# TheIllusionistMirage/libKPEG

Hardware: NVIDIA B200
Metric: decode_mpixel_per_s (higher is better)
Workload: dtype u8/int16 entropy decode, f32 IDCT (f64 on the exact path)

## Files before the change

### libkpeg_b200/csrc/k3_fused.cu

```cuda
#include <cuda_runtime.h>
#include <stddef.h>
#include <stdint.h>

#include <algorithm>
#include <utility>

#include "entropy_core.h"
#include "idct_core.h"
#include "kernels.cuh"
#include "kpeg_common.h"

namespace kpeg {

template <int NAT>
struct NatZz {
    static constexpr int value = make_zigzag_tables().nat2zz[NAT];
};

#ifndef KPEG_EXACT_SKIP_ZERO
#define KPEG_EXACT_SKIP_ZERO 1
#endif

#ifndef KPEG_EXACT_WIDEN_INT
#define KPEG_EXACT_WIDEN_INT 0
// ... 7 lines not shown
constexpr float COLOUR_SAFE_A = 4.0f * (COLOUR_FAST_RANGE - 8.0f);
constexpr float SAMPLE_SAFE_A = 4.0f * 32000.0f;

constexpr float SAMPLE_MAGIC = RINT_MAGIC + 32768.0f;

__host__ __device__ constexpr int tie_bit(int row, int col) { return ((col & 4) ? 0 : 16) + 15 - (4 * (row & 3) + (col & 3)); }
__device__ __forceinline__ int tie_sample(int w, int b)
{
    const int k = 15 - (b & 15);
    return (4 * w + (k >> 2)) * 8 + ((b & 16) ? 0 : 4) + (k & 3);
}

#ifndef KPEG_IDCT_PREFETCH_AHEAD
#define KPEG_IDCT_PREFETCH_AHEAD 1184
#endif
constexpr uint32_t IDCT_PREFETCH_AHEAD = KPEG_IDCT_PREFETCH_AHEAD;

constexpr int TIE_LIST_CAP = IDCT_TIE_LIST_CAP;
constexpr uint32_t TIE_EMPTY = 0xFFFFFFFFu;

template <int NC>
struct IdctSmem {
    static constexpr int NM = IDCT_MCUS_PER_CTA;
    static constexpr int NB = NM * NC;
    union {
        uint4 coef[NB * 8];
        float4 samp[NC * 8 * 2 * NM];
    };
    float2 qpair[NC][32];
    uint2 tiemask[NB];
    uint16_t ties[TIE_LIST_CAP];
    uint8_t flag[NB];
    uint32_t ntie, any_huge;
    uint32_t img0, by0, bx0, mi0;
    unsigned long long mbar;
};
static_assert(sizeof(IdctSmem<3>) <= (233472 / 8 - 1024), "idct_kernel<3> no longer fits eight CTAs per SM");

struct F2 {
    unsigned long long v;
};
__device__ __forceinline__ F2 pack2(float lo, float hi)
{
    F2 r;
    asm("mov.b64 %0, {%1, %2};" : "=l"(r.v) : "f"(lo), "f"(hi));
    return r;
}
__device__ __forceinline__ void unpack2(F2 a, float &lo, float &hi) { asm("mov.b64 {%0, %1}, %2;" : "=f"(lo), "=f"(hi) : "l"(a.v)); }
__device__ __forceinline__ float lo2(F2 a)
{
    float lo, hi;
    unpack2(a, lo, hi);
    return lo;
}
__device__ __forceinline__ float hi2(F2 a)
{
    float lo, hi;
    unpack2(a, lo, hi);
    return hi;
}
__device__ __forceinline__ F2 splat2(float k) { return pack2(k, k); }
__device__ __forceinline__ F2 lane_add(F2 a, F2 b)
{
    F2 r;
    asm("add.rn.f32x2 %0, %1, %2;" : "=l"(r.v) : "l"(a.v), "l"(b.v));
    return r;
// ... 277 lines not shown
    asm volatile("st.shared.u16 [%0], %1;" ::"r"(addr), "h"((uint16_t)v) : "memory");
}

template <int NC>
__global__ void __launch_bounds__(NC * IDCT_MCUS_PER_CTA, NC == 3 ? KPEG_IDCT_MIN_CTAS : 16) idct_kernel(IdctArgs a)
{
    constexpr int NM = IDCT_MCUS_PER_CTA;
    constexpr int NB = NM * NC;
    extern __shared__ __align__(128) unsigned char smem_raw[];
    IdctSmem<NC> &sm = *reinterpret_cast<IdctSmem<NC> *>(smem_raw);

    const int t = threadIdx.x;
    const int comp = t / NM;
    const int ml = t % NM;
    const int bl = ml * NC + comp;
    const uint32_t total_mcus = a.g.nimages * a.g.mcus_per_image;
    const uint32_t strip = blockIdx.x;
    const uint32_t mcu0 = strip * NM;
    const uint32_t m = mcu0 + ml;
    const bool active = m < total_mcus;

    const uint32_t bar = smem_u32(&sm.mbar);
    if (t == 0) {
        constexpr uint32_t table_bytes = NC * 64u * 4u, tile_bytes = NB * 128u;
        const char *tile = reinterpret_cast<const char *>(a.tiles) + (size_t)strip * tile_bytes;
        mbar_init(bar, 1);
        mbar_expect_tx(bar, table_bytes + tile_bytes);
        bulk_load(smem_u32(sm.coef), tile, tile_bytes, bar);
        bulk_load(smem_u32(sm.qpair), a.tables->qpair, table_bytes, bar);
        if (strip + IDCT_PREFETCH_AHEAD < a.nstrips)
            asm volatile("cp.async.bulk.prefetch.L2.global [%0], %1;" ::"l"(tile + (size_t)IDCT_PREFETCH_AHEAD * tile_bytes), "r"(tile_bytes) : "memory");
        sm.ntie = 0;
        sm.any_huge = 0;
        const uint32_t img = mcu0 / a.g.mcus_per_image, mi = mcu0 - img * a.g.mcus_per_image;
        sm.img0 = img;
        sm.mi0 = mi;
        sm.by0 = mi / a.g.mcus_x;
        sm.bx0 = mi - sm.by0 * a.g.mcus_x;
        mbar_wait(bar, 0);
    }
    __syncthreads();

    uint4 ch[8];
#pragma unroll
    for (int k = 0; k < 8; ++k)
        ch[k] = sm.coef[bl * 8 + (k ^ (bl & 7))];
    __syncthreads();
    uint32_t tie_lo = 0, tie_hi = 0;
    if (active) {
        F2 P[32];
        float a_ac, a_dc;
        dequant_dezigzag(ch, sm.qpair[comp], P, a_ac, a_dc, std::make_integer_sequence<int, 32>{});
        const float A = a_ac + a_dc;
        uint32_t flag = (A != 0.0f ? BLK_NONZERO : 0u) | (A > COLOUR_SAFE_A ? BLK_WIDE : 0u);
        if (A > SAMPLE_SAFE_A) {
            flag |= BLK_HUGE;
            sm.any_huge = 1u;
        } else if (a_ac == 0.0f) {
            const int dcv = (int)(ch[0].x & 0xFFFFu) - (int)COEF_BIAS;
            const int F = dcv * __ldg(&a.tables->qint[comp][0]);
            const float tt = mul_f32(__ldg(&a.tables->cc[0][0]), (float)F);
            const float b = (float)round_half_away(0.25f * tt);
            const float4 row = make_float4(b, b, b, b);
#pragma unroll
            for (int i = 0; i < 16; ++i)
                sm.samp[(comp * 16 + i) * NM + ml] = row;
// ... 124 lines not shown
            uint8_t *dst = img_base + ((size_t)y * W + bx * 8u) * NC;
            if (vec_ok) {
#pragma unroll
                for (int k = 0; k < NC; ++k)
                    reinterpret_cast<uint2 *>(dst)[k] = make_uint2(out[2 * k], out[2 * k + 1]);
            } else {
                const uint32_t nbytes = (full_w ? 8u : W - bx * 8u) * NC;
#pragma unroll
                for (int j = 0; j < 8 * NC; ++j)
                    if ((uint32_t)j < nbytes)
                        dst[j] = (uint8_t)(out[j >> 2] >> (8 * (j & 3)));
            }
            while (redo) {
                const int j = __ffs((int)redo) - 1;
                redo &= redo - 1u;
                if (bx * 8u + (uint32_t)j >= W)
                    continue;
                const float *sp = reinterpret_cast<const float *>(sm.samp);
                const int sy = (int)sp[(((0 * 8 + row) * 2 + (j >> 2)) * NM + ml) * 4 + (j & 3)];
                const int sb = (int)sp[(((1 * 8 + row) * 2 + (j >> 2)) * NM + ml) * 4 + (j & 3)];
                const int sr = (int)sp[((((NC - 1) * 8 + row) * 2 + (j >> 2)) * NM + ml) * 4 + (j & 3)];
                const uint32_t e = colour_exact_int(sy, sb, sr);
                dst[3 * j] = (uint8_t)e;
                dst[3 * j + 1] = (uint8_t)(e >> 8);
                dst[3 * j + 2] = (uint8_t)(e >> 16);
                ++colour_exact;
            }
        }
    }
    __syncthreads();

    const uint32_t ntie = sm.ntie;
    if (ntie == 0u && sm.any_huge == 0u) {
        if (t == 0)
            a.tie_cnt[strip] = 0u;
        if (colour_exact)
            atomicAdd(&a.meta->colour_exact, colour_exact);
        return;
    }
    float *spf = reinterpret_cast<float *>(sm.samp);
    const uint4 *gtiles = reinterpret_cast<const uint4 *>(a.tiles);
    const uint32_t blk0 = mcu0 * (uint32_t)NC;
    auto samp_index = [&](uint32_t c, uint32_t mm_l, int s) {
        return ((((c * 8u + (uint32_t)(s >> 3)) * 2u + (uint32_t)((s & 7) >> 2)) * NM + mm_l) * 4u) + (uint32_t)(s & 3);
    };
    auto resolve = [&](uint32_t b, int s) {
        const uint32_t c = b % NC, mm_l = b / NC;
        const int e = exact_sample_global<NC>(gtiles, a.tables, blk0 + b, c, s);
        spf[samp_index(c, mm_l, s)] = (float)e;
    };
    auto repaint = [&](uint32_t b, int s) {
        const uint32_t mm_l = b / NC;
        if (mcu0 + mm_l >= total_mcus)
            return;
        uint32_t img, by, bx;
        mcu_origin(mm_l, img, by, bx);
        const uint32_t px = bx * 8u + (uint32_t)(s & 7), py = by * 8u + (uint32_t)(s >> 3);
        if (px >= W || py >= H)
            return;
        const int y = (int)spf[samp_index(0, mm_l, s)];
        int cb = 0, cr = 0;
        if (NC == 3) {
            cb = (int)spf[samp_index(1, mm_l, s)];
            cr = (int)spf[samp_index(NC - 1, mm_l, s)];
        }
        const uint32_t v = colour_px<NC>(y, cb, cr);
        uint8_t *dst = a.pixels + ((size_t)img * W * H + (size_t)py * W + px) * NC;
        dst[0] = (uint8_t)v;
        if (NC == 3) {
            dst[1] = (uint8_t)(v >> 8);
            dst[2] = (uint8_t)(v >> 16);
        }
    };
    if (ntie <= (uint32_t)TIE_LIST_CAP) {
        for (uint32_t i = (uint32_t)t; i < ntie; i += (uint32_t)NB) {
            const uint32_t e = sm.ties[i], b = e & 127u, mm_l = b / NC, c = b % NC;
            const int sidx = (int)(e >> 7);
            const int tbit = tie_bit(sidx >> 3, sidx & 7);
            uint32_t flags = 0, huge = 0;
#pragma unroll
            for (int cc = 0; cc < NC; ++cc) {
                const uint2 tm = sm.tiemask[mm_l * NC + cc];
                flags |= ((((sidx >> 3) & 4) ? tm.y : tm.x) >> tbit & 1u) << cc;
                huge |= sm.flag[mm_l * NC + cc];
            }
            uint4 r = make_uint4(TIE_EMPTY, 0, 0, 0);
            uint32_t img, by, bx;
            mcu_origin(mm_l, img, by, bx);
            const uint32_t px = bx * 8u + (uint32_t)(sidx & 7), py = by * 8u + (uint32_t)(sidx >> 3);
            if ((flags & (0u - flags)) == (1u << c) && !(huge & BLK_HUGE) && mcu0 + mm_l < total_mcus && px < W && py < H) {
                r.x = img * W * H + py * W + px;
                r.y = mcu0 + mm_l;
                auto biased = [&](uint32_t c) { return ((uint32_t)(int)spf[samp_index(c, mm_l, sidx)] + COEF_BIAS) & 0xFFFFu; };
                r.z = (uint32_t)sidx | (flags << 8) | (biased(0) << 16);
                r.w = NC == 3 ? biased(1) | (biased(2) << 16) : 0u;
            }
            a.tie_rec[(size_t)strip * TIE_LIST_CAP + i] = r;
        }
        if (t == 0)
            a.tie_cnt[strip] = ntie;
    } else {
        if (t == 0)
            a.tie_cnt[strip] = 0u;
        for (int pass = 0; pass < 2; ++pass) {
            uint32_t lo = tie_lo, hi = tie_hi;
            while (lo | hi) {
                int w, b;
                if (lo) {
                    w = 0;
                    b = __ffs((int)lo) - 1;
                    lo &= lo - 1u;
                } else {
                    w = 1;
                    b = __ffs((int)hi) - 1;
                    hi &= hi - 1u;
                }
                if (pass == 0)
                    resolve((uint32_t)bl, tie_sample(w, b));
                else
                    repaint((uint32_t)bl, tie_sample(w, b));
            }
            __syncthreads();
        }
    }
    if (sm.any_huge) {
        __syncthreads();
        for (uint32_t i = (uint32_t)t; i < (uint32_t)NM * 64u; i += (uint32_t)NB) {
            const uint32_t mm_l = i >> 6;
            const int s = (int)(i & 63u);
            uint32_t fl = 0;
            for (int c = 0; c < NC; ++c)
                fl |= sm.flag[mm_l * NC + c];
            if (!(fl & BLK_HUGE) || mcu0 + mm_l >= total_mcus)
                continue;
            uint32_t img, by, bx;
            mcu_origin(mm_l, img, by, bx);
// ... 8 lines not shown
            dst[0] = (uint8_t)v;
            if (NC == 3) {
                dst[1] = (uint8_t)(v >> 8);
                dst[2] = (uint8_t)(v >> 16);
            }
        }
    }
    if (t == 0)
        atomicAdd(&a.meta->exact_samples, ntie);
    if (colour_exact)
        atomicAdd(&a.meta->colour_exact, colour_exact);
}

template <int NC>
__device__ __noinline__ int exact_sample_global(const uint4 *tiles, const DeviceTables *T, uint32_t gb, uint32_t comp, int s)
{
    uint4 ch[8];
#pragma unroll
    for (int k = 0; k < 8; ++k)
        ch[k] = __ldg(tiles + coef_tile_chunk(gb, (uint32_t)k));
    const int x = s >> 3, y = s & 7;
    double cx[8], cy[8];
#pragma unroll
    for (int k = 0; k < 8; ++k) {
        cx[k] = __ldg(&T->cosd[x][k]);
        cy[k] = __ldg(&T->cosd[y][k]);
    }
    const float sum = exact_terms(ch, T->qint[comp], cx, cy, __ldg(&T->cc[0][0]), __ldg(&T->cc[0][1]),
                                  std::make_integer_sequence<int, 64>{});
    const float out = (float)mul_f64(0.25, (double)sum);
    return round_half_away(out);
}

constexpr int PATCH_WARPS = 8;

template <int NC>
__global__ void __launch_bounds__(PATCH_WARPS * 32) idct_patch_kernel(IdctArgs a)
{
    const uint32_t lane = threadIdx.x & 31u, wl = threadIdx.x >> 5;
    const uint4 *tiles = reinterpret_cast<const uint4 *>(a.tiles);
    for (uint32_t s0 = blockIdx.x * 32u; s0 < a.nstrips; s0 += gridDim.x * 32u) {
        const uint32_t strip = s0 + lane;
        const uint32_t cnt = strip < a.nstrips ? min(__ldg(a.tie_cnt + strip), (uint32_t)TIE_LIST_CAP) : 0u;
        uint32_t incl = cnt;
#pragma unroll
        for (int d = 1; d < 32; d <<= 1) {
            const uint32_t o = __shfl_up_sync(0xffffffffu, incl, d);
            if ((int)lane >= d)
                incl += o;
        }
        const uint32_t total = __shfl_sync(0xffffffffu, incl, 31);
        for (uint32_t e0 = wl * 32u; e0 < total; e0 += PATCH_WARPS * 32u) {
            const uint32_t e = e0 + lane;
            uint32_t lo = 0;
#pragma unroll
            for (int step = 16; step >= 1; step >>= 1) {
                const uint32_t v = __shfl_sync(0xffffffffu, incl, (int)(lo + (uint32_t)step - 1u));
                if (v <= e)
                    lo += (uint32_t)step;
            }
            const uint32_t before = __shfl_sync(0xffffffffu, incl - cnt, (int)min(lo, 31u));
            if (e >= total)
                continue;
            const uint4 r = __ldg(a.tie_rec + (size_t)(s0 + lo) * TIE_LIST_CAP + (e - before));
            if (r.x == TIE_EMPTY)
                continue;
            const int s = (int)(r.z & 63u);
            const uint32_t flags = (r.z >> 8) & 7u;
            int v[3] = {(int)(r.z >> 16) - (int)COEF_BIAS, (int)(r.w & 0xFFFFu) - (int)COEF_BIAS, (int)(r.w >> 16) - (int)COEF_BIAS};
            for (uint32_t left = flags; left != 0u; left &= left - 1u) {
                const uint32_t c = (uint32_t)__ffs((int)left) - 1u;
                const int ex = exact_sample_global<NC>(tiles, a.tables, r.y * NC + c, c, s);
                v[0] = c == 0u ? ex : v[0];
                v[1] = c == 1u ? ex : v[1];
                v[2] = c == 2u ? ex : v[2];
            }
            const uint32_t px = colour_px<NC>(v[0], v[1], v[2]);
            uint8_t *dst = a.pixels + (size_t)r.x * NC;
            dst[0] = (uint8_t)px;
            if (NC == 3) {
                dst[1] = (uint8_t)(px >> 8);
                dst[2] = (uint8_t)(px >> 16);
            }
        }
    }
}

void k3_configure()
{
    cudaFuncSetAttribute(idct_kernel<3>, cudaFuncAttributeMaxDynamicSharedMemorySize, (int)sizeof(IdctSmem<3>));
    cudaFuncSetAttribute(idct_kernel<1>, cudaFuncAttributeMaxDynamicSharedMemorySize, (int)sizeof(IdctSmem<1>));
}

uint32_t k3_strip_slots(uint32_t ncomp) { return (uint32_t)IDCT_MCUS_PER_CTA * ncomp * 64u; }

cudaError_t launch_idct(const IdctArgs &a_in, cudaStream_t s, uint32_t *launches)
{
    IdctArgs a = a_in;
    const uint32_t total_mcus = a.g.nimages * a.g.mcus_per_image;
    const uint32_t grid = (total_mcus + IDCT_MCUS_PER_CTA - 1) / IDCT_MCUS_PER_CTA;
    if (a.g.ncomp == 3)
        idct_kernel<3><<<grid, 3 * IDCT_MCUS_PER_CTA, sizeof(IdctSmem<3>), s>>>(a);
    else
        idct_kernel<1><<<grid, IDCT_MCUS_PER_CTA, sizeof(IdctSmem<1>), s>>>(a);
    ++*launches;
    const uint32_t pgrid = std::min<uint32_t>((grid + 31u) / 32u, 148u * 16u);
    if (a.g.ncomp == 3)
        idct_patch_kernel<3><<<pgrid, PATCH_WARPS * 32, 0, s>>>(a);
    else
        idct_patch_kernel<1><<<pgrid, PATCH_WARPS * 32, 0, s>>>(a);
    ++*launches;
    return cudaSuccess;
}

}
```

### libkpeg_b200/csrc/kernels.cuh

```cuda
#ifndef KPEG_KERNELS_CUH
#define KPEG_KERNELS_CUH

#include <cuda_runtime.h>

#include "kpeg_common.h"

namespace kpeg {

constexpr int MAX_RELAY_ROUNDS = 64;

inline int relay_slot(int r) { return r < MAX_RELAY_ROUNDS ? r : 2 + ((r - 2) % (MAX_RELAY_ROUNDS - 2)); }

struct DevMeta {
    uint32_t total_kept;
    uint32_t total_rst;
    uint32_t total_bits;
    uint32_t nsub;
    uint32_t status;
    uint32_t exact_samples;
    uint32_t colour_exact;
    uint32_t final_slot;
    uint32_t reserved_[2];
    uint32_t relay_rounds;
    uint32_t grid_bar;
    uint32_t rec_alt_count;
    uint32_t changed[MAX_RELAY_ROUNDS];
};

struct UnstuffArgs {
    const uint8_t *scan;
    uint32_t scan_len;
    uint32_t ntiles;
    uint32_t *tile_kept, *tile_rst;
    uint32_t *cls;
    uint8_t *words;
    uint32_t *seg_bit;
    uint32_t nseg;
    DevMeta *meta;
};

constexpr int UNSTUFF_THREADS = 256;
constexpr int UNSTUFF_BYTES_PER_THREAD = 16;
constexpr int UNSTUFF_TILE = UNSTUFF_THREADS * UNSTUFF_BYTES_PER_THREAD;

struct EntropyArgs {
    const uint32_t *words;
    const uint32_t *seg_bit;
    const DeviceTables *tables;
    DevMeta *meta;
    SubState *state;
    uint32_t *worklist[2];
    uint32_t *seg_hint;
    uint32_t *start_slot;
    uint2 *scan_tiles;
    long long *scan_tiles_dcs;
// ... 9 lines not shown
    uint32_t *strip_sub;
    uint32_t strip_slots;
    uint32_t nstrips;
    uint32_t nsub_max;
    JobGeom g;
};

constexpr int ENTROPY_THREADS = 128;

constexpr int IDCT_MCUS_PER_CTA = 32;
KPEG_HD uint32_t coef_tile_chunk(uint32_t block, uint32_t k) { return block * 8u + (k ^ (block & 7u)); }
KPEG_HD uint32_t coef_tile_byte(uint32_t slot) { return (slot * 2u) ^ ((slot >> 2) & 0x70u); }

struct ExpandArgs {
    const uint32_t *rec;
    const uint32_t *nrec;
    const uint32_t *rec_alt;
    uint32_t rec_kmax;
    const uint32_t *start_slot;
    const uint32_t *strip_sub;
    const long long *dcpre;
    void *tiles;
    uint32_t nstrips;
    DevMeta *meta;
    JobGeom g;
};

struct IdctArgs {
    const void *tiles;
    uint32_t nstrips;
    const DeviceTables *tables;
    uint8_t *pixels;
    uint4 *tie_rec;
    uint32_t *tie_cnt;
    DevMeta *meta;
    JobGeom g;
};
constexpr int IDCT_TIE_LIST_CAP = 96;


void kernels_context_created();
void kernels_context_destroyed();
void kernels_configure(int max_concurrent_jobs);
void launch_repack_scans(const uint8_t *stage, uint8_t *scan, const uint64_t *ends, uint32_t n, cudaStream_t s);
void launch_write_separators(uint8_t *scan, const uint64_t *ends, uint32_t n, cudaStream_t s);
void launch_count_restart_markers(const uint8_t *scan, uint32_t len, uint32_t *count, cudaStream_t s);
void launch_gray_to_rgb(const uint8_t *gray, uint8_t *rgb, size_t npixels, cudaStream_t s);
void launch_rgb_to_planar(const uint8_t *rgb, uint8_t *planes, size_t npixels, cudaStream_t s);
void launch_unstuff(const UnstuffArgs &a, uint32_t sub_bits, cudaStream_t s, uint32_t *launches);
void launch_entropy_cold(const EntropyArgs &a, cudaStream_t s, uint32_t *launches);
void launch_entropy_relay(const EntropyArgs &a, int round, cudaStream_t s, uint32_t *launches);
cudaError_t launch_entropy_relay_loop(const EntropyArgs &a, int first, int last, cudaStream_t s, uint32_t *launches);
void launch_entropy_scan(const EntropyArgs &a, cudaStream_t s, uint32_t *launches);
void launch_entropy_write(const EntropyArgs &a, cudaStream_t s, uint32_t *launches);
void launch_dc_integrate(const JobGeom &g, const int16_t *dcdiff, int16_t *dc, cudaStream_t s, uint32_t *launches);
void launch_expand(const ExpandArgs &a, cudaStream_t s, uint32_t *launches);
void launch_tiles_from_matrix(const JobGeom &g, const int16_t *coef, const int16_t *dc, void *tiles, cudaStream_t s, uint32_t *launches);
void launch_matrix_from_tiles(const void *tiles, int16_t *coef, uint32_t total_blocks, cudaStream_t s);
void launch_interleave_tiles(const void *t0, const void *t1, const void *t2, void *out, uint32_t nmcu_padded, cudaStream_t s,
                             uint32_t *launches);
cudaError_t launch_idct(const IdctArgs &a, cudaStream_t s, uint32_t *launches);
void k3_configure();
uint32_t k3_strip_slots(uint32_t ncomp);

}
#endif
```

### libkpeg_b200/csrc/kpeg_cuda.cu

```cuda
#include <cuda_runtime.h>
#include <math.h>
#include <stdio.h>
#include <stdlib.h>
#include <string.h>

#include <algorithm>
#include <string>
#include <vector>

#include "host_tables.h"
#include "kernels.cuh"
#include "kpeg_common.h"
#include "kpeg_cuda.h"

using namespace kpeg;

namespace {

struct DevBuf {
    void *p = nullptr;
    size_t cap = 0;
    void *raw = nullptr;
};

// ... 4 lines not shown
    void *p = nullptr;
    size_t cap = 0;
};

constexpr int MAX_EVENTS = 192;
constexpr int NLANES = 8;

struct Copy {
    void *dst;
    const void *src;
    size_t bytes;
    int peer = -1;
};

struct Job {
    bool active = false;
    JobGeom g = {};
    EntropyArgs ea = {};
    ExpandArgs xa = {};
    IdctArgs ia = {};
    int rounds = 0;
    uint32_t launches = 0;
    uint32_t extra_iterations = 0;
    bool use_records = true;
    bool loop_used = true;
    size_t scan_len = 0;
    std::vector<Copy> d2h;
    bool entropy_only = false;
};

struct Lane {
    cudaStream_t stream = nullptr;
    DevBuf scan, words, seg_bit, tile_kept, tile_rst, cls, state, work, seg_hint, start_slot, scan_tiles;
    DevBuf coef, dcdiff, dc, tiles, tie_rec, tie_cnt, pixels, meta, rec, nrec, rec_alt, strip_sub, dcs, dcpre, scan_tiles_dcs;
    PinBuf h_meta;
    PinBuf h_stage, h_ends;
    DevBuf d_ends, d_stage;
    cudaEvent_t ev[MAX_EVENTS] = {};
    int ev_stage[MAX_EVENTS] = {};
    int nev = 0;
    Job job;
};

}

struct kpeg_ctx {
    int device = 0;
    std::string err;
    bool profiling = false;
    uint32_t sub_bits = 512;
    bool sub_bits_auto = true;
    int relay_rounds = 8;
    bool use_records = true;
    int split_parts = 4;
    int host_chunks = 8;
    int submit_parts = 1;
    int band_parts = 4;
    DevBuf band_counts;
    PinBuf h_band_counts;
    bool relay_round2_wide = false;
    bool d2h_chain = true;
    bool d2h_chain_armed = false;
    cudaEvent_t d2h_done = nullptr;
    Lane lane[NLANES];

    DevBuf tables, merged;
    DevBuf scan_tiles[3];
// ... 273 lines not shown
        const uint64_t bits = (uint64_t)scan_len * 8u;
        sub_bits = (bits >= segs * ((uint64_t)4 << 20) && bits >= blocks * 96u) ? 1024u : 512u;
    }
    int rc = make_job_geom(pl, nimages, sub_bits, &g, &why);
    if (rc != KPEG_OK)
        return fail(ctx, rc, why);
    if (scan_len == 0 || scan_len >= (1ull << 29))
        return fail(ctx, KPEG_ERR_ARG, "entropy-coded segment must be 1 byte .. 512 MiB");
    TRY(upload_plan(ctx, pl));

    const uint32_t S = (uint32_t)scan_len;
    const uint32_t ntiles = (S + 15u + UNSTUFF_TILE - 1) / UNSTUFF_TILE;
    const uint32_t nsub_max = (uint32_t)(((uint64_t)S * 8u + g.sub_bits - 1u) / g.sub_bits) + 1u;
    const uint32_t total_mcus = g.nimages * g.mcus_per_image;
    const uint32_t nstrips = (total_mcus + IDCT_MCUS_PER_CTA - 1) / IDCT_MCUS_PER_CTA;
    const size_t words_bytes = ((size_t)S + 3u) / 4u * 4u + 64u;

    TRY(ensure(ctx, s, L.words, words_bytes));
    TRY(ensure(ctx, s, L.seg_bit, ((size_t)g.nseg + 2u) * 4u));
    TRY(ensure(ctx, s, L.tile_kept, (size_t)ntiles * 4u));
    TRY(ensure(ctx, s, L.tile_rst, (size_t)ntiles * 4u));
    TRY(ensure(ctx, s, L.cls, (size_t)ntiles * UNSTUFF_THREADS * 4u));
    TRY(ensure(ctx, s, L.state, (size_t)nsub_max * sizeof(SubState)));
    TRY(ensure(ctx, s, L.work, (size_t)nsub_max * 2u * sizeof(uint32_t)));
    TRY(ensure(ctx, s, L.seg_hint, (size_t)nsub_max * 4u));
    TRY(ensure(ctx, s, L.start_slot, (size_t)nsub_max * 4u));
    TRY(ensure(ctx, s, L.scan_tiles, ((size_t)nsub_max / 1024u + 2u) * sizeof(uint2)));
    TRY(ensure(ctx, s, L.strip_sub, ((size_t)nstrips + 1u) * sizeof(uint32_t)));
    TRY(ensure(ctx, s, L.dcs, (size_t)nsub_max * sizeof(long long)));
    TRY(ensure(ctx, s, L.dcpre, (size_t)nsub_max * sizeof(long long)));
    TRY(ensure(ctx, s, L.scan_tiles_dcs, ((size_t)nsub_max / 1024u + 2u) * sizeof(long long)));
    TRY(ensure(ctx, s, L.tiles, (size_t)nstrips * IDCT_MCUS_PER_CTA * g.ncomp * 128u + 256u));
    TRY(ensure(ctx, s, L.tie_rec, (size_t)nstrips * IDCT_TIE_LIST_CAP * sizeof(uint4)));
    TRY(ensure(ctx, s, L.tie_cnt, (size_t)nstrips * sizeof(uint32_t)));
    TRY(ensure(ctx, s, L.meta, sizeof(DevMeta)));
    TRY(ensure_pinned(ctx, s, L.h_meta, sizeof(DevMeta)));
    const uint32_t rec_kmax = (g.sub_bits * 3u / 8u + 7u) & ~7u;
    const uint32_t rec_alt_cap = nsub_max / 4u + 1024u;
    if (ctx->use_records) {
        TRY(ensure(ctx, s, L.rec, (size_t)rec_kmax * ((size_t)nsub_max / 32u + 1u) * 32u * sizeof(uint32_t)));
        TRY(ensure(ctx, s, L.nrec, (size_t)nsub_max * sizeof(uint32_t)));
        TRY(ensure(ctx, s, L.rec_alt, (size_t)rec_alt_cap * rec_kmax * sizeof(uint32_t)));
    }

    J = Job();
    J.use_records = ctx->use_records && ctx->plan_fits_records;
    J.active = true;
    J.g = g;
    J.scan_len = scan_len;
    J.d2h = std::move(d2h);
    J.entropy_only = tiles_only != nullptr;
    void *const tiles = tiles_only ? tiles_only : L.tiles.p;
    DevMeta *d_meta = (DevMeta *)L.meta.p;

    CK(cudaMemsetAsync(d_meta, 0, sizeof(DevMeta), s));
    mark(ctx, L, KPEG_T_MEMSET);

    UnstuffArgs ua;
    ua.scan = d_scan;
    ua.scan_len = S;
    ua.ntiles = ntiles;
    ua.tile_kept = (uint32_t *)L.tile_kept.p;
    ua.tile_rst = (uint32_t *)L.tile_rst.p;
    ua.cls = (uint32_t *)L.cls.p;
    ua.words = (uint8_t *)L.words.p;
    ua.seg_bit = (uint32_t *)L.seg_bit.p;
    ua.nseg = g.nseg;
// ... 17 lines not shown
    ea.dcpre = (long long *)L.dcpre.p;
    ea.rec = J.use_records ? (uint32_t *)L.rec.p : nullptr;
    ea.nrec = (uint32_t *)L.nrec.p;
    ea.rec_kmax = rec_kmax;
    ea.rec_alt = (uint32_t *)L.rec_alt.p;
    ea.rec_alt_cap = rec_alt_cap;
    ea.coef = nullptr;
    ea.dcdiff = nullptr;
    ea.strip_sub = (uint32_t *)L.strip_sub.p;
    ea.strip_slots = k3_strip_slots(g.ncomp);
    ea.nstrips = nstrips;
    ea.nsub_max = nsub_max;
    ea.g = g;

    ExpandArgs &xa = J.xa;
    xa.rec = ea.rec;
    xa.nrec = ea.nrec;
    xa.rec_alt = ea.rec_alt;
    xa.rec_kmax = rec_kmax;
    xa.start_slot = ea.start_slot;
    xa.strip_sub = ea.strip_sub;
    xa.dcpre = ea.dcpre;
    xa.tiles = tiles;
    xa.nstrips = nstrips;
    xa.meta = d_meta;
    xa.g = g;

    IdctArgs &ia = J.ia;
    ia.tiles = tiles;
    ia.nstrips = nstrips;
    ia.tables = (const DeviceTables *)ctx->tables.p;
    ia.pixels = d_pixels;
    ia.tie_rec = (uint4 *)L.tie_rec.p;
    ia.tie_cnt = (uint32_t *)L.tie_cnt.p;
    ia.meta = d_meta;
    ia.g = g;

    launch_entropy_cold(ea, s, &J.launches);
    mark(ctx, L, KPEG_T_ENTROPY_COLD);
    J.rounds = ctx->relay_rounds < 2 ? 2 : (ctx->relay_rounds > MAX_RELAY_ROUNDS - 1 ? MAX_RELAY_ROUNDS - 1 : ctx->relay_rounds);
    launch_entropy_relay(ea, 1, s, &J.launches);
    mark(ctx, L, KPEG_T_ENTROPY_RELAY);
    if (ctx->relay_round2_wide)
        launch_entropy_relay(ea, 2, s, &J.launches);
    const int loop_first = ctx->relay_round2_wide ? 3 : 2;
    J.rounds = MAX_RELAY_ROUNDS - 2;
    if (launch_entropy_relay_loop(ea, loop_first, J.rounds, s, &J.launches) != cudaSuccess) {
        J.loop_used = false;
        J.rounds = std::max(loop_first, std::min(ctx->relay_rounds, MAX_RELAY_ROUNDS - 1));
        for (int r = loop_first; r <= J.rounds; ++r)
            launch_entropy_relay(ea, r, s, &J.launches);
    }
    mark(ctx, L, KPEG_T_RELAY_SPARSE);
    return enqueue_downstream(ctx, L);
}

struct NamedBuf {
    const char *name;
    DevBuf *buf;
};

int check_guards(kpeg_ctx *ctx, Lane &L)
{
    NamedBuf bufs[] = {{"cls", &L.cls},           {"scan", &L.scan},         {"words", &L.words},       {"seg_bit", &L.seg_bit},
                       {"tile_kept", &L.tile_kept}, {"tile_rst", &L.tile_rst}, {"state", &L.state},       {"work", &L.work},
                       {"seg_hint", &L.seg_hint}, {"start_slot", &L.start_slot}, {"scan_tiles", &L.scan_tiles},
                       {"coef", &L.coef},         {"dcdiff", &L.dcdiff},     {"tiles", &L.tiles},       {"tie_rec", &L.tie_rec},   {"tie_cnt", &L.tie_cnt},     {"strip_sub", &L.strip_sub}, {"dc", &L.dc}, {"dcs", &L.dcs}, {"dcpre", &L.dcpre}, {"scan_tiles_dcs", &L.scan_tiles_dcs}, {"d_ends", &L.d_ends},
                       {"pixels", &L.pixels},     {"meta", &L.meta},
                       {"rec", &L.rec},           {"nrec", &L.nrec},         {"rec_alt", &L.rec_alt},   {"tables", &ctx->tables},
                       {"d_stage", &L.d_stage},   {"scan_tiles[0]", &ctx->scan_tiles[0]}, {"scan_tiles[1]", &ctx->scan_tiles[1]},
                       {"scan_tiles[2]", &ctx->scan_tiles[2]}, {"band_counts", &ctx->band_counts}, {"merged", &ctx->merged}};
    uint8_t host[2 * GUARD_BYTES];
    for (const NamedBuf &nb : bufs) {
        const DevBuf &b = *nb.buf;
        if (!b.raw || b.raw == b.p)
            continue;
        CK(cudaMemcpy(host, b.raw, GUARD_BYTES, cudaMemcpyDeviceToHost));
        CK(cudaMemcpy(host + GUARD_BYTES, (const uint8_t *)b.p + b.cap, GUARD_BYTES, cudaMemcpyDeviceToHost));
        for (size_t i = 0; i < 2 * GUARD_BYTES; ++i)
            if (host[i] != (uint8_t)GUARD_PATTERN) {
                char msg[160];
                snprintf(msg, sizeof msg, "guard bytes %s device buffer '%s' (%zu bytes) were overwritten at offset %zu",
                         i < GUARD_BYTES ? "before" : "after", nb.name, b.cap, i % GUARD_BYTES);
                return fail(ctx, KPEG_ERR_CUDA, msg);
            }
    }
    return KPEG_OK;
}

int job_finish(kpeg_ctx *ctx, int li, kpeg_stats *stats)
{
    Lane &L = ctx->lane[li];
    Job &J = L.job;
    if (!J.active)
        return KPEG_OK;
    J.active = false;
    cudaStream_t s = L.stream;
    DevMeta *d_meta = (DevMeta *)L.meta.p;
    DevMeta *h_meta = (DevMeta *)L.h_meta.p;
    for (;;) {
        CK(cudaStreamSynchronize(s));
        CK(cudaGetLastError());
        if (h_meta->status & (ST_BAD_MARKER | ST_SEG_COUNT))
            break;
        const bool timed_out = (h_meta->status & ST_RELAY_TIMEOUT) != 0u;
        if (J.extra_iterations == 0u && J.loop_used)
            J.rounds = (int)std::max<uint32_t>(h_meta->relay_rounds, 1u);
        const bool converged_now = !timed_out && h_meta->changed[relay_slot(J.rounds)] == 0u;
        if (converged_now && J.use_records && (h_meta->status & ST_REC_OVERFLOW)) {
            J.use_records = false;
            CK(cudaMemsetAsync(&d_meta->status, 0, sizeof(uint32_t), s));
            CK(cudaMemsetAsync(&d_meta->exact_samples, 0, 2 * sizeof(uint32_t), s));
            TRY(enqueue_downstream(ctx, L));
            continue;
        }
        if (converged_now)
            break;
        bool converged = false;
        bool repeat = timed_out;
        const uint32_t cap = h_meta->nsub / 2u + 4u;
        while (!converged && J.extra_iterations < cap) {
            ++J.extra_iterations;
            for (int k = 0; k < 2; ++k) {
                ++J.rounds;
                if (!repeat)
                    CK(cudaMemsetAsync(&d_meta->changed[relay_slot(J.rounds)], 0, sizeof(uint32_t), s));
                repeat = false;
                launch_entropy_relay(J.ea, J.rounds, s, &J.launches);
            }
            mark(ctx, L, KPEG_T_RELAY_SPARSE);
            CK(cudaMemcpyAsync(h_meta, d_meta, sizeof(DevMeta), cudaMemcpyDeviceToHost, s));
            CK(cudaStreamSynchronize(s));
            converged = h_meta->changed[relay_slot(J.rounds)] == 0u;
        }
        if (!converged)
            return fail(ctx, KPEG_ERR_NOT_CONVERGED, "speculative decode did not reach a fixed point");
        CK(cudaMemsetAsync(&d_meta->status, 0, sizeof(uint32_t), s));
        CK(cudaMemsetAsync(&d_meta->exact_samples, 0, 2 * sizeof(uint32_t), s));
        TRY(enqueue_downstream(ctx, L));
    }
    if (ctx->guard)
        TRY(check_guards(ctx, L));
    ctx->last_lane = li;
    ctx->last_g = J.g;
    if (stats) {
        stats->width = J.g.width;
        stats->height = J.g.height;
        stats->ncomp = J.g.ncomp;
        stats->scan_bytes += J.scan_len;
        stats->unstuffed_bytes += h_meta->total_kept;
        stats->segments += h_meta->total_rst + 1u;
        stats->subsequences += h_meta->nsub;
        uint32_t used_rounds = (uint32_t)J.rounds;
        if (J.extra_iterations == 0u) {
            used_rounds = 0;
            for (int r = 1; r <= J.rounds && r < MAX_RELAY_ROUNDS; ++r)
                if (h_meta->changed[r])
                    used_rounds = (uint32_t)r;
        }
        stats->sync_rounds = std::max(stats->sync_rounds, used_rounds);
        stats->exact_samples += h_meta->exact_samples;
        stats->kernel_launches += J.launches;
        add_times(ctx, L, stats);
    }
    return status_to_rc(ctx, h_meta->status & ~(ST_REC_OVERFLOW | ST_RELAY_TIMEOUT));
}

void zero_stats(kpeg_stats *stats)
{
    if (stats)
        memset(stats, 0, sizeof *stats);
// ... 160 lines not shown
    if (const char *rr = getenv("KPEG_RELAY_ROUNDS")) {
        const long v = strtol(rr, nullptr, 10);
        if (v >= 2 && v < MAX_RELAY_ROUNDS)
            ctx->relay_rounds = (int)v;
    }
    cudaMallocHost(&ctx->h_sep.p, 64);
    if (ctx->h_sep.p) {
        ctx->h_sep.cap = 64;
        uint8_t *sep = (uint8_t *)ctx->h_sep.p;
        for (int k = 0; k < 8; ++k) {
            sep[2 * k] = 0xFF;
            sep[2 * k + 1] = (uint8_t)(0xD0 + k);
        }
    }
    if (cudaGetLastError() != cudaSuccess || !ctx->h_sep.p) {
        kpeg_cuda_destroy(ctx);
        return KPEG_ERR_CUDA;
    }
    *out = ctx;
    return KPEG_OK;
}

extern "C" void kpeg_cuda_destroy(kpeg_ctx *ctx)
{
    if (!ctx)
        return;
    cudaSetDevice(ctx->device);
    if (ctx->counted)
        kernels_context_destroyed();
    for (Lane &L : ctx->lane) {
        if (L.stream)
            cudaStreamSynchronize(L.stream);
        DevBuf *bufs[] = {&L.cls,  &L.scan, &L.words,    &L.seg_bit,    &L.tile_kept,  &L.tile_rst, &L.state,
                          &L.work, &L.seg_hint, &L.start_slot, &L.scan_tiles, &L.coef,     &L.dcdiff, &L.tiles, &L.tie_rec, &L.tie_cnt,
                          &L.strip_sub, &L.dc, &L.dcs, &L.dcpre, &L.scan_tiles_dcs, &L.pixels, &L.meta,
                          &L.rec,  &L.nrec,       &L.rec_alt};
        for (DevBuf *b : bufs)
            dev_free(*b);
        if (L.h_meta.p)
            cudaFreeHost(L.h_meta.p);
        if (L.h_stage.p)
            cudaFreeHost(L.h_stage.p);
        if (L.h_ends.p)
            cudaFreeHost(L.h_ends.p);
        dev_free(L.d_ends);
        dev_free(L.d_stage);
        for (int i = 0; i < MAX_EVENTS; ++i)
            if (L.ev[i])
                cudaEventDestroy(L.ev[i]);
        if (L.stream)
            cudaStreamDestroy(L.stream);
    }
    dev_free(ctx->tables);
    dev_free(ctx->merged);
    if (ctx->h_tables.p)
        cudaFreeHost(ctx->h_tables.p);
    if (ctx->h_sep.p)
        cudaFreeHost(ctx->h_sep.p);
    if (ctx->tables_ready)
        cudaEventDestroy(ctx->tables_ready);
    if (ctx->d2h_done)
        cudaEventDestroy(ctx->d2h_done);
    for (DevBuf &b : ctx->scan_tiles)
        dev_free(b);
    dev_free(ctx->band_counts);
    if (ctx->h_band_counts.p)
        cudaFreeHost(ctx->h_band_counts.p);
// ... 535 lines not shown
        kpeg_plan pl = scans[k].plan;
        pl.flags = frame->flags;
        TRY(ensure(ctx, s, L.scan, scans[k].len + 64));
        mark(ctx, L, -1);
        CK(cudaMemcpyAsync(L.scan.p, file + scans[k].off, scans[k].len, cudaMemcpyHostToDevice, s));
        mark(ctx, L, KPEG_T_H2D);
        TRY(job_enqueue(ctx, 0, &pl, (const uint8_t *)L.scan.p, scans[k].len, 1, nullptr, {}, ctx->scan_tiles[scans[k].comp[0]].p));
        memset(&part, 0, sizeof part);
        TRY(job_finish(ctx, 0, stats ? &part : nullptr));
        if (stats) {
            stats->scan_bytes += part.scan_bytes;
            stats->unstuffed_bytes += part.unstuffed_bytes;
            stats->segments += part.segments;
            stats->subsequences += part.subsequences;
            stats->sync_rounds = std::max(stats->sync_rounds, part.sync_rounds);
            stats->kernel_launches += part.kernel_launches;
            for (int t = 0; t < KPEG_T_COUNT; ++t)
                stats->ms[t] += part.ms[t];
            stats->ms_total += part.ms_total;
        }
    }
    kpeg_plan fp = *frame;
    for (int c = 0; c < 3; ++c) {
        fp.comp_td[c] = scans[0].plan.comp_td[0];
        fp.comp_ta[c] = scans[0].plan.comp_ta[0];
    }
    memcpy(fp.ht, scans[0].plan.ht, sizeof fp.ht);
    memcpy(fp.ht_present, scans[0].plan.ht_present, sizeof fp.ht_present);
    TRY(upload_plan(ctx, &fp));
    const size_t npix = (size_t)frame->width * frame->height * 3u;
    TRY(ensure(ctx, s, L.tiles, (size_t)nmcu_padded * 3u * 128u + 256u));
    TRY(ensure(ctx, s, L.pixels, npix + 64));
    TRY(ensure(ctx, s, L.tie_rec, (size_t)nstrips * IDCT_TIE_LIST_CAP * sizeof(uint4)));
    TRY(ensure(ctx, s, L.tie_cnt, (size_t)nstrips * sizeof(uint32_t)));
    DevMeta *d_meta = (DevMeta *)L.meta.p, *h_meta = (DevMeta *)L.h_meta.p;
    CK(cudaMemsetAsync(d_meta, 0, sizeof(DevMeta), s));
    mark(ctx, L, -1);
    launch_interleave_tiles(ctx->scan_tiles[0].p, ctx->scan_tiles[1].p, ctx->scan_tiles[2].p, L.tiles.p, nmcu_padded, s, &launches);
    IdctArgs ia;
    ia.tiles = L.tiles.p;
    ia.nstrips = nstrips;
    ia.tables = (const DeviceTables *)ctx->tables.p;
    ia.pixels = (uint8_t *)L.pixels.p;
    ia.tie_rec = (uint4 *)L.tie_rec.p;
    ia.tie_cnt = (uint32_t *)L.tie_cnt.p;
    ia.meta = d_meta;
    ia.g = g3;
    CK(launch_idct(ia, s, &launches));
    mark(ctx, L, KPEG_T_IDCT);
    CK(cudaMemcpyAsync(pixels_out, L.pixels.p, npix, cudaMemcpyDeviceToHost, s));
    mark(ctx, L, KPEG_T_D2H);
    CK(cudaMemcpyAsync(h_meta, d_meta, sizeof(DevMeta), cudaMemcpyDeviceToHost, s));
    CK(cudaStreamSynchronize(s));
    CK(cudaGetLastError());
    if (ctx->guard)
        TRY(check_guards(ctx, L));
    ctx->last_lane = 0;
    ctx->last_g = g3;
    if (stats) {
        stats->width = frame->width;
        stats->height = frame->height;
        stats->ncomp = 3;
        stats->exact_samples += h_meta->exact_samples;
        stats->kernel_launches += launches;
        add_times(ctx, L, stats);
    }
    return KPEG_OK;
}

extern "C" int kpeg_cuda_decode_file(kpeg_ctx *ctx, const uint8_t *file, size_t len, uint32_t flags, uint8_t *pixels_out,
                                     size_t cap, kpeg_plan *plan_out, kpeg_stats *stats)
{
    if (!ctx || !file || !pixels_out)
        return KPEG_ERR_ARG;
    kpeg_plan frame;
    kpeg_scan scans[KPEG_MAX_SCANS];
    int nscans = 0;
    const int prc = kpeg_parse_jfif_scans(file, len, &frame, scans, KPEG_MAX_SCANS, &nscans);
// ... 175 lines not shown
```

Measured before the change: 86930.

## Compact tie records via global atomic counter instead of per-strip counts

Each IDCT CTA that has ties now reserves a contiguous range in a global tie-record buffer with one atomicAdd on a new meta counter, instead of writing to a fixed per-strip slot and a per-strip count array. The patch kernel then runs a flat grid-stride loop over only the used records, dropping the per-strip count loads, the warp prefix scan and the binary search over strips. This removes the tie_cnt writes from every strip and the scan over all strips in the patch pass, at the cost of an atomic plus an extra barrier for strips with ties. The patch grid is now sized from buffer capacity rather than strip count, and the exact_samples memset widens to clear the new counter.

```diff
diff --git a/libkpeg_b200/csrc/k3_fused.cu b/libkpeg_b200/csrc/k3_fused.cu
--- a/libkpeg_b200/csrc/k3_fused.cu
+++ b/libkpeg_b200/csrc/k3_fused.cu
@@ -63,6 +63,7 @@
     uint16_t ties[TIE_LIST_CAP];
     uint8_t flag[NB];
     uint32_t ntie, any_huge;
+    uint32_t rec0;
     uint32_t img0, by0, bx0, mi0;
     unsigned long long mbar;
 };
@@ -406,6 +407,7 @@
             asm volatile("cp.async.bulk.prefetch.L2.global [%0], %1;" ::"l"(tile + (size_t)IDCT_PREFETCH_AHEAD * tile_bytes), "r"(tile_bytes) : "memory");
         sm.ntie = 0;
         sm.any_huge = 0;
+        sm.rec0 = 0;
         const uint32_t img = mcu0 / a.g.mcus_per_image, mi = mcu0 - img * a.g.mcus_per_image;
         sm.img0 = img;
         sm.mi0 = mi;
@@ -596,8 +598,6 @@
 
     const uint32_t ntie = sm.ntie;
     if (ntie == 0u && sm.any_huge == 0u) {
-        if (t == 0)
-            a.tie_cnt[strip] = 0u;
         if (colour_exact)
             atomicAdd(&a.meta->colour_exact, colour_exact);
         return;
@@ -636,7 +636,13 @@
             dst[2] = (uint8_t)(v >> 16);
         }
     };
-    if (ntie <= (uint32_t)TIE_LIST_CAP) {
+    if (ntie <= (uint32_t)TIE_LIST_CAP && ntie != 0u) {
+        if (t == 0)
+            sm.rec0 = atomicAdd(&a.meta->tie_records, ntie);
+        __syncthreads();
+    }
+    const uint32_t rec0 = sm.rec0;
+    if (ntie <= (uint32_t)TIE_LIST_CAP && rec0 + ntie <= a.tie_cap) {
         for (uint32_t i = (uint32_t)t; i < ntie; i += (uint32_t)NB) {
             const uint32_t e = sm.ties[i], b = e & 127u, mm_l = b / NC, c = b % NC;
             const int sidx = (int)(e >> 7);
@@ -659,13 +665,12 @@
                 r.z = (uint32_t)sidx | (flags << 8) | (biased(0) << 16);
                 r.w = NC == 3 ? biased(1) | (biased(2) << 16) : 0u;
             }
-            a.tie_rec[(size_t)strip * TIE_LIST_CAP + i] = r;
-        }
-        if (t == 0)
-            a.tie_cnt[strip] = ntie;
+            a.tie_rec[rec0 + i] = r;
+        }
     } else {
-        if (t == 0)
-            a.tie_cnt[strip] = 0u;
+        if (ntie <= (uint32_t)TIE_LIST_CAP)
+            for (uint32_t i = rec0 + (uint32_t)t; i < a.tie_cap && i < rec0 + ntie; i += (uint32_t)NB)
+                a.tie_rec[i] = make_uint4(TIE_EMPTY, 0, 0, 0);
         for (int pass = 0; pass < 2; ++pass) {
             uint32_t lo = tie_lo, hi = tie_hi;
             while (lo | hi) {
@@ -740,56 +745,33 @@
     return round_half_away(out);
 }
 
-constexpr int PATCH_WARPS = 8;
+constexpr int PATCH_THREADS = 256;
 
 template <int NC>
-__global__ void __launch_bounds__(PATCH_WARPS * 32) idct_patch_kernel(IdctArgs a)
-{
-    const uint32_t lane = threadIdx.x & 31u, wl = threadIdx.x >> 5;
+__global__ void __launch_bounds__(PATCH_THREADS) idct_patch_kernel(IdctArgs a)
+{
     const uint4 *tiles = reinterpret_cast<const uint4 *>(a.tiles);
-    for (uint32_t s0 = blockIdx.x * 32u; s0 < a.nstrips; s0 += gridDim.x * 32u) {
-        const uint32_t strip = s0 + lane;
-        const uint32_t cnt = strip < a.nstrips ? min(__ldg(a.tie_cnt + strip), (uint32_t)TIE_LIST_CAP) : 0u;
-        uint32_t incl = cnt;
-#pragma unroll
-        for (int d = 1; d < 32; d <<= 1) {
-            const uint32_t o = __shfl_up_sync(0xffffffffu, incl, d);
-            if ((int)lane >= d)
-                incl += o;
-        }
-        const uint32_t total = __shfl_sync(0xffffffffu, incl, 31);
-        for (uint32_t e0 = wl * 32u; e0 < total; e0 += PATCH_WARPS * 32u) {
-            const uint32_t e = e0 + lane;
-            uint32_t lo = 0;
-#pragma unroll
-            for (int step = 16; step >= 1; step >>= 1) {
-                const uint32_t v = __shfl_sync(0xffffffffu, incl, (int)(lo + (uint32_t)step - 1u));
-                if (v <= e)
-                    lo += (uint32_t)step;
-            }
-            const uint32_t before = __shfl_sync(0xffffffffu, incl - cnt, (int)min(lo, 31u));
-            if (e >= total)
-                continue;
-            const uint4 r = __ldg(a.tie_rec + (size_t)(s0 + lo) * TIE_LIST_CAP + (e - before));
-            if (r.x == TIE_EMPTY)
-                continue;
-            const int s = (int)(r.z & 63u);
-            const uint32_t flags = (r.z >> 8) & 7u;
-            int v[3] = {(int)(r.z >> 16) - (int)COEF_BIAS, (int)(r.w & 0xFFFFu) - (int)COEF_BIAS, (int)(r.w >> 16) - (int)COEF_BIAS};
-            for (uint32_t left = flags; left != 0u; left &= left - 1u) {
-                const uint32_t c = (uint32_t)__ffs((int)left) - 1u;
-                const int ex = exact_sample_global<NC>(tiles, a.tables, r.y * NC + c, c, s);
-                v[0] = c == 0u ? ex : v[0];
-                v[1] = c == 1u ? ex : v[1];
-                v[2] = c == 2u ? ex : v[2];
-            }
-            const uint32_t px = colour_px<NC>(v[0], v[1], v[2]);
-            uint8_t *dst = a.pixels + (size_t)r.x * NC;
-            dst[0] = (uint8_t)px;
-            if (NC == 3) {
-                dst[1] = (uint8_t)(px >> 8);
-                dst[2] = (uint8_t)(px >> 16);
-            }
+    const uint32_t n = min(a.meta->tie_records, a.tie_cap);
+    for (uint32_t i = blockIdx.x * PATCH_THREADS + threadIdx.x; i < n; i += gridDim.x * PATCH_THREADS) {
+        const uint4 r = __ldg(a.tie_rec + i);
+        if (r.x == TIE_EMPTY)
+            continue;
+        const int s = (int)(r.z & 63u);
+        const uint32_t flags = (r.z >> 8) & 7u;
+        int v[3] = {(int)(r.z >> 16) - (int)COEF_BIAS, (int)(r.w & 0xFFFFu) - (int)COEF_BIAS, (int)(r.w >> 16) - (int)COEF_BIAS};
+        for (uint32_t left = flags; left != 0u; left &= left - 1u) {
+            const uint32_t c = (uint32_t)__ffs((int)left) - 1u;
+            const int ex = exact_sample_global<NC>(tiles, a.tables, r.y * NC + c, c, s);
+            v[0] = c == 0u ? ex : v[0];
+            v[1] = c == 1u ? ex : v[1];
+            v[2] = c == 2u ? ex : v[2];
+        }
+        const uint32_t px = colour_px<NC>(v[0], v[1], v[2]);
+        uint8_t *dst = a.pixels + (size_t)r.x * NC;
+        dst[0] = (uint8_t)px;
+        if (NC == 3) {
+            dst[1] = (uint8_t)(px >> 8);
+            dst[2] = (uint8_t)(px >> 16);
         }
     }
 }
@@ -812,11 +794,11 @@
     else
         idct_kernel<1><<<grid, IDCT_MCUS_PER_CTA, sizeof(IdctSmem<1>), s>>>(a);
     ++*launches;
-    const uint32_t pgrid = std::min<uint32_t>((grid + 31u) / 32u, 148u * 16u);
+    const uint32_t pgrid = std::max<uint32_t>(1u, std::min<uint32_t>((a.tie_cap + PATCH_THREADS - 1u) / PATCH_THREADS, 148u * 8u));
     if (a.g.ncomp == 3)
-        idct_patch_kernel<3><<<pgrid, PATCH_WARPS * 32, 0, s>>>(a);
+        idct_patch_kernel<3><<<pgrid, PATCH_THREADS, 0, s>>>(a);
     else
-        idct_patch_kernel<1><<<pgrid, PATCH_WARPS * 32, 0, s>>>(a);
+        idct_patch_kernel<1><<<pgrid, PATCH_THREADS, 0, s>>>(a);
     ++*launches;
     return cudaSuccess;
 }
diff --git a/libkpeg_b200/csrc/kernels.cuh b/libkpeg_b200/csrc/kernels.cuh
--- a/libkpeg_b200/csrc/kernels.cuh
+++ b/libkpeg_b200/csrc/kernels.cuh
@@ -19,8 +19,9 @@
     uint32_t status;
     uint32_t exact_samples;
     uint32_t colour_exact;
+    uint32_t tie_records;
     uint32_t final_slot;
-    uint32_t reserved_[2];
+    uint32_t reserved_[1];
     uint32_t relay_rounds;
     uint32_t grid_bar;
     uint32_t rec_alt_count;
@@ -96,7 +97,7 @@
     const DeviceTables *tables;
     uint8_t *pixels;
     uint4 *tie_rec;
-    uint32_t *tie_cnt;
+    uint32_t tie_cap;
     DevMeta *meta;
     JobGeom g;
 };
diff --git a/libkpeg_b200/csrc/kpeg_cuda.cu b/libkpeg_b200/csrc/kpeg_cuda.cu
--- a/libkpeg_b200/csrc/kpeg_cuda.cu
+++ b/libkpeg_b200/csrc/kpeg_cuda.cu
@@ -60,7 +60,7 @@
 struct Lane {
     cudaStream_t stream = nullptr;
     DevBuf scan, words, seg_bit, tile_kept, tile_rst, cls, state, work, seg_hint, start_slot, scan_tiles;
-    DevBuf coef, dcdiff, dc, tiles, tie_rec, tie_cnt, pixels, meta, rec, nrec, rec_alt, strip_sub, dcs, dcpre, scan_tiles_dcs;
+    DevBuf coef, dcdiff, dc, tiles, tie_rec, pixels, meta, rec, nrec, rec_alt, strip_sub, dcs, dcpre, scan_tiles_dcs;
     PinBuf h_meta;
     PinBuf h_stage, h_ends;
     DevBuf d_ends, d_stage;
@@ -400,7 +400,6 @@
     TRY(ensure(ctx, s, L.scan_tiles_dcs, ((size_t)nsub_max / 1024u + 2u) * sizeof(long long)));
     TRY(ensure(ctx, s, L.tiles, (size_t)nstrips * IDCT_MCUS_PER_CTA * g.ncomp * 128u + 256u));
     TRY(ensure(ctx, s, L.tie_rec, (size_t)nstrips * IDCT_TIE_LIST_CAP * sizeof(uint4)));
-    TRY(ensure(ctx, s, L.tie_cnt, (size_t)nstrips * sizeof(uint32_t)));
     TRY(ensure(ctx, s, L.meta, sizeof(DevMeta)));
     TRY(ensure_pinned(ctx, s, L.h_meta, sizeof(DevMeta)));
     const uint32_t rec_kmax = (g.sub_bits * 3u / 8u + 7u) & ~7u;
@@ -484,7 +483,7 @@
     ia.tables = (const DeviceTables *)ctx->tables.p;
     ia.pixels = d_pixels;
     ia.tie_rec = (uint4 *)L.tie_rec.p;
-    ia.tie_cnt = (uint32_t *)L.tie_cnt.p;
+    ia.tie_cap = (uint32_t)(L.tie_rec.cap / sizeof(uint4));
     ia.meta = d_meta;
     ia.g = g;
 
@@ -517,7 +516,7 @@
     NamedBuf bufs[] = {{"cls", &L.cls},           {"scan", &L.scan},         {"words", &L.words},       {"seg_bit", &L.seg_bit},
                        {"tile_kept", &L.tile_kept}, {"tile_rst", &L.tile_rst}, {"state", &L.state},       {"work", &L.work},
                        {"seg_hint", &L.seg_hint}, {"start_slot", &L.start_slot}, {"scan_tiles", &L.scan_tiles},
-                       {"coef", &L.coef},         {"dcdiff", &L.dcdiff},     {"tiles", &L.tiles},       {"tie_rec", &L.tie_rec},   {"tie_cnt", &L.tie_cnt},     {"strip_sub", &L.strip_sub}, {"dc", &L.dc}, {"dcs", &L.dcs}, {"dcpre", &L.dcpre}, {"scan_tiles_dcs", &L.scan_tiles_dcs}, {"d_ends", &L.d_ends},
+                       {"coef", &L.coef},         {"dcdiff", &L.dcdiff},     {"tiles", &L.tiles},       {"tie_rec", &L.tie_rec},     {"strip_sub", &L.strip_sub}, {"dc", &L.dc}, {"dcs", &L.dcs}, {"dcpre", &L.dcpre}, {"scan_tiles_dcs", &L.scan_tiles_dcs}, {"d_ends", &L.d_ends},
                        {"pixels", &L.pixels},     {"meta", &L.meta},
                        {"rec", &L.rec},           {"nrec", &L.nrec},         {"rec_alt", &L.rec_alt},   {"tables", &ctx->tables},
                        {"d_stage", &L.d_stage},   {"scan_tiles[0]", &ctx->scan_tiles[0]}, {"scan_tiles[1]", &ctx->scan_tiles[1]},
@@ -562,7 +561,7 @@
         if (converged_now && J.use_records && (h_meta->status & ST_REC_OVERFLOW)) {
             J.use_records = false;
             CK(cudaMemsetAsync(&d_meta->status, 0, sizeof(uint32_t), s));
-            CK(cudaMemsetAsync(&d_meta->exact_samples, 0, 2 * sizeof(uint32_t), s));
+            CK(cudaMemsetAsync(&d_meta->exact_samples, 0, 3 * sizeof(uint32_t), s));
             TRY(enqueue_downstream(ctx, L));
             continue;
         }
@@ -588,7 +587,7 @@
         if (!converged)
             return fail(ctx, KPEG_ERR_NOT_CONVERGED, "speculative decode did not reach a fixed point");
         CK(cudaMemsetAsync(&d_meta->status, 0, sizeof(uint32_t), s));
-        CK(cudaMemsetAsync(&d_meta->exact_samples, 0, 2 * sizeof(uint32_t), s));
+        CK(cudaMemsetAsync(&d_meta->exact_samples, 0, 3 * sizeof(uint32_t), s));
         TRY(enqueue_downstream(ctx, L));
     }
     if (ctx->guard)
@@ -815,7 +814,7 @@
         if (L.stream)
             cudaStreamSynchronize(L.stream);
         DevBuf *bufs[] = {&L.cls,  &L.scan, &L.words,    &L.seg_bit,    &L.tile_kept,  &L.tile_rst, &L.state,
-                          &L.work, &L.seg_hint, &L.start_slot, &L.scan_tiles, &L.coef,     &L.dcdiff, &L.tiles, &L.tie_rec, &L.tie_cnt,
+                          &L.work, &L.seg_hint, &L.start_slot, &L.scan_tiles, &L.coef,     &L.dcdiff, &L.tiles, &L.tie_rec,
                           &L.strip_sub, &L.dc, &L.dcs, &L.dcpre, &L.scan_tiles_dcs, &L.pixels, &L.meta,
                           &L.rec,  &L.nrec,       &L.rec_alt};
         for (DevBuf *b : bufs)
@@ -1417,7 +1416,6 @@
     TRY(ensure(ctx, s, L.tiles, (size_t)nmcu_padded * 3u * 128u + 256u));
     TRY(ensure(ctx, s, L.pixels, npix + 64));
     TRY(ensure(ctx, s, L.tie_rec, (size_t)nstrips * IDCT_TIE_LIST_CAP * sizeof(uint4)));
-    TRY(ensure(ctx, s, L.tie_cnt, (size_t)nstrips * sizeof(uint32_t)));
     DevMeta *d_meta = (DevMeta *)L.meta.p, *h_meta = (DevMeta *)L.h_meta.p;
     CK(cudaMemsetAsync(d_meta, 0, sizeof(DevMeta), s));
     mark(ctx, L, -1);
@@ -1428,7 +1426,7 @@
     ia.tables = (const DeviceTables *)ctx->tables.p;
     ia.pixels = (uint8_t *)L.pixels.p;
     ia.tie_rec = (uint4 *)L.tie_rec.p;
-    ia.tie_cnt = (uint32_t *)L.tie_cnt.p;
+    ia.tie_cap = (uint32_t)(L.tie_rec.cap / sizeof(uint4));
     ia.meta = d_meta;
     ia.g = g3;
     CK(launch_idct(ia, s, &launches));
```

Result: no change. 86330 (median of 6 runs) (-0.7%).
